# xiexh20/CHORE

Hardware: AMD Instinct MI355X
Metric: query-points/sec (HGFilters encode + 20k-pt MLP field query per 512x512 image) (higher is better)
Workload: dtype fp16x3; 1 GPU; BASELINE configs[1]: encode 4x(5,512,512) + query 4x20000 points per GPU per step; images_per_gpu=4, points_per_image=20000, batches_in_flight=2

## Files before the change

### chore_amd/csrc/query_fwd.hip

```cpp
#include "heads_x3.h"
#include <cstdlib>

template <int PTS>
struct QueryFwdSmemT {
    float X[PTS * XS];
    PtTableT<PTS> tab;
};
using QueryFwdSmem = QueryFwdSmemT<QT_PTS>;

template <typename T, int NCB, bool TRAIN = false, bool X3 = false>
__global__ __launch_bounds__(256, 1) void query_fwd_f32_kernel(QueryArgs a) {
    static_assert(!TRAIN || NCB == 2, "the training staging is written for 64-point tiles");
    constexpr int PTS = 32 * NCB;
    if constexpr (X3) f16_saturate_mode();
    extern __shared__ __attribute__((aligned(16))) char smem_raw[];
    QueryFwdSmemT<PTS>& sm = *reinterpret_cast<QueryFwdSmemT<PTS>*>(smem_raw);
    const int tid = threadIdx.x, lane = tid & 63;
    const int wid = __builtin_amdgcn_readfirstlane(tid >> 6);
    int b, tile_;
    query_block(b, tile_);
    const int n0 = tile_ * PTS;
    const Cam cam{a.fx, a.fy, a.cx, a.cy, a.half_crop, a.crop};

    if (tid < PTS) {
        fill_pt_table(sm.tab, tid, a.points, a.crop_center, b, n0 + tid, a.N, cam, a.FH, a.FW, a.TH,
                      a.TW, nullptr);
        if (a.in_img && n0 + tid < a.N) a.in_img[(size_t)b * a.N + n0 + tid] = (uint8_t)sm.tab.in_img[tid];
    }
    __syncthreads();
    const T* feat_b = (const T*)a.feat + (size_t)b * a.FH * a.FW * FEAT_C;
    const T* tmpx_b = (const T*)a.tmpx + (size_t)b * a.TH * a.TW * TMPX_C;
    gather_tile<T, PTS>(sm.X, sm.tab, feat_b, tmpx_b, wid, lane);
    __syncthreads();

    const float* arena = (const float*)a.arena;
    const int head = wid;
    if constexpr (!TRAIN) {
        if (a.out[head] == nullptr) return;
    }
    f32x16 h1[4][NCB], h2[4][NCB];
    const size_t row0 = (size_t)b * a.N + n0, plane = (size_t)a.B * a.N * HEAD_HID, mplane = (size_t)a.B * a.N * 2;
    if constexpr (TRAIN) {
        for (int i = tid; i < PTS * (QF_KPAD / 4); i += 256) {
            const int pt = i / (QF_KPAD / 4), q = i % (QF_KPAD / 4);
            if (n0 + pt < a.N) *(f32x4*)(a.tX + (row0 + pt) * QF_KPAD + 4 * q) = *(const f32x4*)(sm.X + pt * XS + 4 * q);
        }
    }
    f32x16 o[NCB];
    if constexpr (X3) {
        float inv[NCB];
#pragma unroll
        for (int cb = 0; cb < NCB; ++cb) inv[cb] = QX_INV;
        heads_layer1_x3<NCB>(h1, sm.X, arena, head, lane);
        if constexpr (TRAIN) store_tile<NCB>(a.tH + (0 * HEAD_NUM + head) * plane, h1, true, row0, n0, a.N, lane, 0, inv);
        if constexpr (TRAIN) store_masks<NCB>(a.tM + (0 * HEAD_NUM + head) * mplane, h1, row0, n0, a.N, lane, 0);
        heads_layer_hid_x3<NCB>(h2, h1, arena, head, 1, lane);
        if constexpr (TRAIN) store_tile<NCB>(a.tH + (1 * HEAD_NUM + head) * plane, h2, true, row0, n0, a.N, lane, 0, inv);
        if constexpr (TRAIN) store_masks<NCB>(a.tM + (1 * HEAD_NUM + head) * mplane, h2, row0, n0, a.N, lane, 0);
        heads_layer_hid_x3<NCB>(h1, h2, arena, head, 2, lane);
        if constexpr (TRAIN) store_tile<NCB>(a.tH + (2 * HEAD_NUM + head) * plane, h1, true, row0, n0, a.N, lane, 0, inv);
        if constexpr (TRAIN) store_masks<NCB>(a.tM + (2 * HEAD_NUM + head) * mplane, h1, row0, n0, a.N, lane, 0);
        heads_layer_out_x3<NCB>(o, h1, arena, head, lane);
    } else {
        heads_layer1<NCB>(h1, sm.X, arena, head, lane);
        if constexpr (TRAIN) store_tile<NCB>(a.tH + (0 * HEAD_NUM + head) * plane, h1, true, row0, n0, a.N, lane);
        if constexpr (TRAIN) store_masks<NCB>(a.tM + (0 * HEAD_NUM + head) * mplane, h1, row0, n0, a.N, lane);
        heads_layer_hid<NCB>(h2, h1, arena, head, 1, lane);
        if constexpr (TRAIN) store_tile<NCB>(a.tH + (1 * HEAD_NUM + head) * plane, h2, true, row0, n0, a.N, lane);
        if constexpr (TRAIN) store_masks<NCB>(a.tM + (1 * HEAD_NUM + head) * mplane, h2, row0, n0, a.N, lane);
        heads_layer_hid<NCB>(h1, h2, arena, head, 2, lane);
        if constexpr (TRAIN) store_tile<NCB>(a.tH + (2 * HEAD_NUM + head) * plane, h1, true, row0, n0, a.N, lane);
        if constexpr (TRAIN) store_masks<NCB>(a.tM + (2 * HEAD_NUM + head) * mplane, h1, row0, n0, a.N, lane);
        heads_layer_out<NCB>(o, h1, arena, head, lane);
    }

    const int odim = head_out_dim(head);
    float* outp = a.out[head] + (size_t)b * odim * a.N;
    const int half = lane >> 5, col = lane & 31;
#pragma unroll
    for (int cb = 0; cb < NCB; ++cb) {
        const int pt = cb * 32 + col;
        const int n = n0 + pt;
        const bool inside = sm.tab.in_img[pt] != 0;
#pragma unroll
        for (int r = 0; r < 16; ++r) {
            const int ch = mfma32_row(r, half);
            if (ch < odim && n < a.N) {
                float v = o[cb][r];
                if (head == 0 && !inside) v = 5.0f;
                outp[(size_t)ch * a.N + n] = v;
            }
        }
    }
}

template <typename T, bool TRAIN = false, bool X3 = false>
__global__ __launch_bounds__(512, 1) void query_fwd_f32_w8_kernel(QueryArgs a) {
    constexpr int PTS = 64;
    if constexpr (X3) f16_saturate_mode();
    extern __shared__ __attribute__((aligned(16))) char smem_raw[];
    QueryFwdSmemT<PTS>& sm = *reinterpret_cast<QueryFwdSmemT<PTS>*>(smem_raw);
    const int tid = threadIdx.x, lane = tid & 63;
    const int wid = __builtin_amdgcn_readfirstlane(tid >> 6);
    float* scr = reinterpret_cast<float*>(smem_raw + sizeof(QueryFwdSmemT<PTS>)) + wid * (32 * ST_LD);
    int b, tile_;
    query_block(b, tile_);
    const int n0 = tile_ * PTS;
    const Cam cam{a.fx, a.fy, a.cx, a.cy, a.half_crop, a.crop};
    if (tid < PTS) {
        fill_pt_table(sm.tab, tid, a.points, a.crop_center, b, n0 + tid, a.N, cam, a.FH, a.FW, a.TH,
                      a.TW, nullptr);
        if (a.in_img && n0 + tid < a.N) a.in_img[(size_t)b * a.N + n0 + tid] = (uint8_t)sm.tab.in_img[tid];
    }
    __syncthreads();
    const T* feat_b = (const T*)a.feat + (size_t)b * a.FH * a.FW * FEAT_C;
    const T* tmpx_b = (const T*)a.tmpx + (size_t)b * a.TH * a.TW * TMPX_C;
    gather_tile<T, PTS, 8>(sm.X, sm.tab, feat_b, tmpx_b, wid, lane);
    __syncthreads();

    const float* arena = (const float*)a.arena;
    const int head = wid & 3, cb0 = wid >> 2;
    if constexpr (!TRAIN) {
        if (a.out[head] == nullptr) return;
    }
    f32x16 h1[4][1], h2[4][1];
    const size_t row0 = (size_t)b * a.N + n0, plane = (size_t)a.B * a.N * HEAD_HID, mplane = (size_t)a.B * a.N * 2;
    if constexpr (TRAIN) {
        for (int i = tid; i < PTS * (QF_KPAD / 4); i += 512) {
            const int pt = i / (QF_KPAD / 4), q = i % (QF_KPAD / 4);
            if (n0 + pt < a.N) *(f32x4*)(a.tX + (row0 + pt) * QF_KPAD + 4 * q) = *(const f32x4*)(sm.X + pt * XS + 4 * q);
        }
    }
    f32x16 o[1];
    if constexpr (X3) {
        const float inv[1] = {QX_INV};
        heads_layer1_x3<1>(h1, sm.X + cb0 * 32 * XS, arena, head, lane);
        if constexpr (TRAIN) store_tile_lds<1>(a.tH + (0 * HEAD_NUM + head) * plane, h1, true, row0, n0, a.N, lane, cb0 * 32, inv, scr);
        if constexpr (TRAIN) store_masks<1>(a.tM + (0 * HEAD_NUM + head) * mplane, h1, row0, n0, a.N, lane, cb0 * 32);
        heads_layer_hid_x3<1>(h2, h1, arena, head, 1, lane);
        if constexpr (TRAIN) store_tile_lds<1>(a.tH + (1 * HEAD_NUM + head) * plane, h2, true, row0, n0, a.N, lane, cb0 * 32, inv, scr);
        if constexpr (TRAIN) store_masks<1>(a.tM + (1 * HEAD_NUM + head) * mplane, h2, row0, n0, a.N, lane, cb0 * 32);
        heads_layer_hid_x3<1>(h1, h2, arena, head, 2, lane);
        if constexpr (TRAIN) store_tile_lds<1>(a.tH + (2 * HEAD_NUM + head) * plane, h1, true, row0, n0, a.N, lane, cb0 * 32, inv, scr);
        if constexpr (TRAIN) store_masks<1>(a.tM + (2 * HEAD_NUM + head) * mplane, h1, row0, n0, a.N, lane, cb0 * 32);
        heads_layer_out_x3<1>(o, h1, arena, head, lane);
    } else {
        heads_layer1<1>(h1, sm.X + cb0 * 32 * XS, arena, head, lane);
        if constexpr (TRAIN) store_tile_lds<1>(a.tH + (0 * HEAD_NUM + head) * plane, h1, true, row0, n0, a.N, lane, cb0 * 32, nullptr, scr);
        if constexpr (TRAIN) store_masks<1>(a.tM + (0 * HEAD_NUM + head) * mplane, h1, row0, n0, a.N, lane, cb0 * 32);
        heads_layer_hid<1>(h2, h1, arena, head, 1, lane);
        if constexpr (TRAIN) store_tile_lds<1>(a.tH + (1 * HEAD_NUM + head) * plane, h2, true, row0, n0, a.N, lane, cb0 * 32, nullptr, scr);
        if constexpr (TRAIN) store_masks<1>(a.tM + (1 * HEAD_NUM + head) * mplane, h2, row0, n0, a.N, lane, cb0 * 32);
        heads_layer_hid<1>(h1, h2, arena, head, 2, lane);
        if constexpr (TRAIN) store_tile_lds<1>(a.tH + (2 * HEAD_NUM + head) * plane, h1, true, row0, n0, a.N, lane, cb0 * 32, nullptr, scr);
        if constexpr (TRAIN) store_masks<1>(a.tM + (2 * HEAD_NUM + head) * mplane, h1, row0, n0, a.N, lane, cb0 * 32);
        heads_layer_out<1>(o, h1, arena, head, lane);
    }

    const int odim = head_out_dim(head);
    float* outp = a.out[head] + (size_t)b * odim * a.N;
    const int half = lane >> 5, col = lane & 31;
    const int pt = cb0 * 32 + col, n = n0 + pt;
    const bool inside = sm.tab.in_img[pt] != 0;
#pragma unroll
    for (int r = 0; r < 16; ++r) {
        const int ch = mfma32_row(r, half);
        if (ch < odim && n < a.N) {
            float v = o[0][r];
            if (head == 0 && !inside) v = 5.0f;
            outp[(size_t)ch * a.N + n] = v;
        }
    }
}

constexpr int XSH = 344;
template <int PTS>
struct QuerySplitSmemT {
    static constexpr size_t XB = (size_t)2 * PTS * XSH * 2;
    static constexpr size_t EB = (size_t)HEAD_NUM * 4 * 2 * (PTS / 32) * 2 * 1024;
    __attribute__((aligned(16))) char buf[XB > EB ? XB : EB];
    PtTableT<PTS> tab;
};

template <typename T, int PTS>
__device__ __forceinline__ void gather_tile_split(char* XH, char* XL, const PtTableT<PTS>& tab, const T* feat_b, const T* tmpx_b,
                                                  int wid, int lane) {
    using L = MapLoad<T>;
    constexpr int NW = 8, U = PTS / NW;
    auto put = [&](char* row_h, char* row_l, int k, float v) {
        asm volatile("" : "+v"(v));
        const _Float16 h = (_Float16)v, l = (_Float16)(v - (float)h);
        *(_Float16*)(row_h + 2 * k) = h;
        *(_Float16*)(row_l + 2 * k) = l;
    };
    typename L::Raw4 fv[U][4];
    typename L::Raw1 tv[U][4];
#pragma unroll
    for (int u = 0; u < U; ++u) {
        const int pt = wid * U + u;
#pragma unroll
        for (int k = 0; k < 4; ++k) {
            const int fo = tab.foff[k][pt];
            const int to = tab.toff[k][pt];
            fv[u][k] = (fo >= 0) ? L::raw4(feat_b + fo + lane * 4) : L::zero4();
            tv[u][k] = (to >= 0) ? L::raw1(tmpx_b + to + lane) : L::zero1();
        }
    }
#pragma unroll
    for (int u = 0; u < U; ++u) {
        const int pt = wid * U + u;
        float fw[4], tw[4];
#pragma unroll
        for (int k = 0; k < 4; ++k) { fw[k] = tab.fw[k][pt]; tw[k] = tab.tw[k][pt]; }
        const f32x4 c0 = L::cvt4(fv[u][0]), c1 = L::cvt4(fv[u][1]), c2 = L::cvt4(fv[u][2]), c3 = L::cvt4(fv[u][3]);
        typedef _Float16 h4 __attribute__((ext_vector_type(4)));
        h4 hh, ll;
#pragma unroll
        for (int c = 0; c < 4; ++c) {
            float r = interp4(c0[c], c1[c], c2[c], c3[c], fw);
            asm volatile("" : "+v"(r));
            hh[c] = (_Float16)r;
            ll[c] = (_Float16)(r - (float)hh[c]);
        }
        char* rh = XH + (size_t)pt * XSH * 2;
        char* rl = XL + (size_t)pt * XSH * 2;
        *(h4*)(rh + lane * 8) = hh;
        *(h4*)(rl + lane * 8) = ll;
        put(rh, rl, FEAT_C + 3 + lane, interp4(L::cvt1(tv[u][0], lane & 1), L::cvt1(tv[u][1], lane & 1), L::cvt1(tv[u][2], lane & 1),
                                               L::cvt1(tv[u][3], lane & 1), tw));
        if (lane < 3) put(rh, rl, FEAT_C + lane, tab.xyz[lane][pt]);
        if (lane >= 3 && lane < 3 + (QX_KS1 * 16 - HEAD_IN)) put(rh, rl, HEAD_IN + lane - 3, 0.f);
    }
}

#ifdef CHORE_QUERY_STAMPS
__device__ unsigned long long g_qstamps[4096 * 8];
#define QSTAMP(i) do { if (tid == 0) { const int L_ = blockIdx.x + blockIdx.y * gridDim.x; if (L_ < 4096) g_qstamps[L_ * 8 + (i)] = wall_clock64(); } } while (0)
__device__ unsigned short g_qx[2 * 64 * XSH];
__device__ int g_qx_tile = -1;
extern "C" int chore_debug_query_xdump(unsigned short* out, int tile) {
    if (tile >= 0) return (int)hipMemcpyToSymbol(HIP_SYMBOL(g_qx_tile), &tile, sizeof(int));
    return (int)hipMemcpyFromSymbol(out, HIP_SYMBOL(g_qx), sizeof(unsigned short) * 2 * 64 * XSH);
}
extern "C" int chore_debug_query_stamps(unsigned long long* out, int n) {
    return (int)hipMemcpyFromSymbol(out, HIP_SYMBOL(g_qstamps), sizeof(unsigned long long) * (n < 4096 * 8 ? n : 4096 * 8));
}
#else
#define QSTAMP(i) do { } while (0)
#endif
struct AFrag2 { u32x4 h[2], l[2]; };
__device__ __forceinline__ void load_afrag2(AFrag2& f, const u32x4* A , int rb0) {
#pragma unroll
    for (int i = 0; i < 2; ++i) { f.h[i] = A[((rb0 + i) * 2) * 64]; f.l[i] = A[((rb0 + i) * 2 + 1) * 64]; }
}

template <typename T, int NCB>
__global__ __launch_bounds__(512, 1) void query_fwd_x3_split_kernel(QueryArgs a) {
    constexpr int PTS = 32 * NCB, PF = 7, NSTEP = QX_KS1 + 16;
    static_assert(QX_KS1 % PF == 0, "the k loop of layer 1 is unrolled by the ring depth");
    f16_saturate_mode();
    extern __shared__ __attribute__((aligned(16))) char smem_raw[];
    QuerySplitSmemT<PTS>& sm = *reinterpret_cast<QuerySplitSmemT<PTS>*>(smem_raw);
    char* XH = sm.buf;
    char* XL = sm.buf + (size_t)PTS * XSH * 2;
    u32x4* E = (u32x4*)sm.buf;
    const int tid = threadIdx.x, lane = tid & 63;
    const int wid = __builtin_amdgcn_readfirstlane(tid >> 6);
    const int half = lane >> 5, col = lane & 31;
    int b, tile_;
    query_block(b, tile_);
    const int n0 = tile_ * PTS;
    const Cam cam{a.fx, a.fy, a.cx, a.cy, a.half_crop, a.crop};
    QSTAMP(0);
    if (tid < PTS) {
        fill_pt_table(sm.tab, tid, a.points, a.crop_center, b, n0 + tid, a.N, cam, a.FH, a.FW, a.TH, a.TW, nullptr, a.perm);
        if (a.in_img && n0 + tid < a.N) a.in_img[(size_t)b * a.N + sm.tab.pidx[tid]] = (uint8_t)sm.tab.in_img[tid];
    }
    __syncthreads();
    QSTAMP(1);
    const float* arena = (const float*)a.arena;
    const int head = wid & 3, ch = wid >> 2, rb0 = 2 * ch;
    const bool active = a.out[head] != nullptr;
    const u32x4* xbase = (const u32x4*)((const char*)arena + QX_OFF_BYTES);
    const u32x4* A1 = xbase + (size_t)head * QX_KS1 * 4 * 2 * 64 + lane;
    const u32x4* A23 = xbase + QX_L1_VEC + (size_t)head * 2 * 4 * 2 * 4 * 2 * 64 + lane;
    auto step_ptr = [&](int st) -> const u32x4* {
        return st < QX_KS1 ? A1 + (size_t)st * 4 * 2 * 64 : A23 + (size_t)(st - QX_KS1) * 4 * 2 * 64;
    };
    AFrag2 ring[PF];
    constexpr bool RING_EARLY = sizeof(T) == 2 || NCB == 1;
    if (RING_EARLY && active) {
#pragma unroll
        for (int p = 0; p < PF; ++p) load_afrag2(ring[p], step_ptr(p), rb0);
    }
    const T* feat_b = (const T*)a.feat + (size_t)b * a.FH * a.FW * FEAT_C;
    const T* tmpx_b = (const T*)a.tmpx + (size_t)b * a.TH * a.TW * TMPX_C;
    gather_tile_split<T, PTS>(XH, XL, sm.tab, feat_b, tmpx_b, wid, lane);
    if (!RING_EARLY && active) {
#pragma unroll
        for (int p = 0; p < PF; ++p) load_afrag2(ring[p], step_ptr(p), rb0);
    }
    __syncthreads();
    QSTAMP(2);
#ifdef CHORE_QUERY_STAMPS
    if (b == 0 && tile_ == g_qx_tile)
        for (int i = tid; i < 2 * PTS * XSH; i += 512) g_qx[i] = ((const unsigned short*)sm.buf)[i];
#endif

    f32x16 acc[2][NCB], nb[2];
    auto mm = [&](const AFrag2& f, const u32x4 (&bh)[NCB], const u32x4 (&bl)[NCB]) {
#pragma unroll
        for (int i = 0; i < 2; ++i)
#pragma unroll
            for (int cb = 0; cb < NCB; ++cb) acc[i][cb] = mfma3(f.h[i], f.l[i], bh[cb], bl[cb], acc[i][cb]);
    };
    auto fetch_bias = [&](int layer) {
#pragma unroll
        for (int i = 0; i < 2; ++i) nb[i] = scaled_bias(arena, head, layer, rb0 + i, half);
    };
    auto init_acc = [&]() {
#pragma unroll
        for (int i = 0; i < 2; ++i)
#pragma unroll
            for (int cb = 0; cb < NCB; ++cb) acc[i][cb] = nb[i];
    };
    auto publish = [&]() {
#pragma unroll
        for (int i = 0; i < 2; ++i)
#pragma unroll
            for (int s = 0; s < 2; ++s)
#pragma unroll
                for (int cb = 0; cb < NCB; ++cb) {
                    float v[8];
#pragma unroll
                    for (int j = 0; j < 8; ++j) v[j] = relu(acc[i][cb][8 * s + j] * QX_INV);
                    u32x4 hi, lo;
                    split8(v, hi, lo);
                    u32x4* dst = E + ((((size_t)(head * 4 + rb0 + i) * 2 + s) * NCB + cb) * 2) * 64 + lane;
                    dst[0] = hi;
                    dst[64] = lo;
                }
    };

    if (active) {
        fetch_bias(0);
        init_acc();
        fetch_bias(1);
        const char* xh0 = XH + (size_t)col * XSH * 2 + 16 * half;
        const char* xl0 = XL + (size_t)col * XSH * 2 + 16 * half;
#pragma unroll 1
        for (int k0 = 0; k0 < QX_KS1; k0 += PF) {
#pragma unroll
            for (int p = 0; p < PF; ++p) {
                const int ks = k0 + p;
                u32x4 bh[NCB], bl[NCB];
#pragma unroll
                for (int cb = 0; cb < NCB; ++cb) {
                    bh[cb] = *(const u32x4*)(xh0 + (size_t)cb * 32 * XSH * 2 + ks * 32);
                    bl[cb] = *(const u32x4*)(xl0 + (size_t)cb * 32 * XSH * 2 + ks * 32);
                }
                mm(ring[p], bh, bl);
                load_afrag2(ring[p], step_ptr(ks + PF), rb0);
                __builtin_amdgcn_sched_barrier(0);
            }
        }
    }
    __syncthreads();
    QSTAMP(3);
    if (active) publish();
    __syncthreads();

    u32x4 ah[8], al[8];
#pragma unroll
    for (int layer = 1; layer <= 2; ++layer) {
        if (active) {
            init_acc();
            fetch_bias(layer + 1);
            const u32x4* Eh = E + (size_t)head * 4 * 2 * NCB * 2 * 64 + lane;
#pragma unroll
            for (int t = 0; t < 8; ++t) {
                const int st = QX_KS1 + 8 * (layer - 1) + t;
                u32x4 bh[NCB], bl[NCB];
#pragma unroll
                for (int cb = 0; cb < NCB; ++cb) {
                    bh[cb] = Eh[((size_t)(t * NCB + cb) * 2) * 64];
                    bl[cb] = Eh[((size_t)(t * NCB + cb) * 2 + 1) * 64];
                }
                mm(ring[st % PF], bh, bl);
                if (st + PF < NSTEP) load_afrag2(ring[st % PF], step_ptr(st + PF), rb0);
                __builtin_amdgcn_sched_barrier(0);
            }
            if (layer == 2) {
                const u32x4* A = xbase + QX_L1_VEC + QX_L23_VEC + (size_t)head * 4 * 2 * 2 * 64 + lane;
#pragma unroll
                for (int t = 0; t < 8; ++t) { ah[t] = A[(t * 2) * 64]; al[t] = A[(t * 2 + 1) * 64]; }
            }
        }
        __syncthreads();
        if (active) publish();
        __syncthreads();
    }

    QSTAMP(4);
    const int cb_o = NCB == 2 ? ch : 0;
    if (!active || (NCB == 1 && ch != 0)) return;
    f32x16 o = nb[0];
    if (rb0 != 0) o = scaled_bias(arena, head, 3, 0, half);
    {
        const u32x4* Eh = E + (size_t)head * 4 * 2 * NCB * 2 * 64 + lane;
#pragma unroll
        for (int t = 0; t < 8; ++t) {
            const u32x4 bh = Eh[((size_t)(t * NCB + cb_o) * 2) * 64], bl = Eh[((size_t)(t * NCB + cb_o) * 2 + 1) * 64];
            o = mfma3(ah[t], al[t], bh, bl, o);
        }
    }
    const int odim = head_out_dim(head);
    float* outp = a.out[head] + (size_t)b * odim * a.N;
    const int pt = cb_o * 32 + col, n = sm.tab.pidx[pt];
    const bool inside = sm.tab.in_img[pt] != 0;
#pragma unroll
    for (int r = 0; r < 16; ++r) {
        const int chn = mfma32_row(r, half);
        if (chn < odim && n0 + pt < a.N) {
            float v = o[r] * QX_INV;
            if (head == 0 && !inside) v = 5.0f;
            outp[(size_t)chn * a.N + n] = v;
        }
    }
    QSTAMP(5);
}

template <typename T, int NCB>
static int launch_query_fwd_split(chore_handle* h, const QueryArgs& a, hipStream_t s) {
    constexpr int PTS = 32 * NCB;
    const size_t smem = sizeof(QuerySplitSmemT<PTS>);
    dim3 grid((a.N + PTS - 1) / PTS, a.B);
    return CHORE_LAUNCH(h, s, (query_fwd_x3_split_kernel<T, NCB>), grid, dim3(512), smem, a);
}

template <typename T>
__global__ __launch_bounds__(256) void sample_features_kernel(QueryArgs a, float* features, float* nxy) {
    extern __shared__ __attribute__((aligned(16))) char smem_raw[];
    QueryFwdSmem& sm = *reinterpret_cast<QueryFwdSmem*>(smem_raw);
    const int tid = threadIdx.x, lane = tid & 63;
    const int wid = __builtin_amdgcn_readfirstlane(tid >> 6);
    int b, tile_;
    query_block(b, tile_);
    const int n0 = tile_ * QT_PTS;
    const Cam cam{a.fx, a.fy, a.cx, a.cy, a.half_crop, a.crop};
    if (tid < QT_PTS) {
        float nn[2];
        fill_pt_table(sm.tab, tid, a.points, a.crop_center, b, n0 + tid, a.N, cam, a.FH, a.FW, a.TH, a.TW, nn);
        if (nxy && n0 + tid < a.N) {
            nxy[((size_t)b * a.N + n0 + tid) * 2 + 0] = nn[0];
            nxy[((size_t)b * a.N + n0 + tid) * 2 + 1] = nn[1];
        }
        if (a.in_img && n0 + tid < a.N) a.in_img[(size_t)b * a.N + n0 + tid] = (uint8_t)sm.tab.in_img[tid];
    }
    __syncthreads();
    const T* feat_b = (const T*)a.feat + (size_t)b * a.FH * a.FW * FEAT_C;
    const T* tmpx_b = (const T*)a.tmpx + (size_t)b * a.TH * a.TW * TMPX_C;
    gather_tile<T>(sm.X, sm.tab, feat_b, tmpx_b, wid, lane);
    __syncthreads();
    for (int i = tid; i < QT_PTS * HEAD_IN; i += 256) {
        const int pt = i / HEAD_IN, k = i % HEAD_IN;
        if (n0 + pt < a.N) features[((size_t)b * a.N + n0 + pt) * HEAD_IN + k] = sm.X[pt * XS + k];
    }
}

template <typename T>
static int launch_sample_features_t(chore_handle* h, const QueryArgs& a, float* features, float* nxy, hipStream_t s) {
    const size_t smem = sizeof(QueryFwdSmem);
    dim3 grid((a.N + QT_PTS - 1) / QT_PTS, a.B);
    return CHORE_LAUNCH(h, s, sample_features_kernel<T>, grid, dim3(256), smem, a, features, nxy);
}
int launch_sample_features(chore_handle* h, int dtype, const QueryArgs& a, float* features, float* nxy, hipStream_t s) {
    return dtype == CHORE_F32 ? launch_sample_features_t<float>(h, a, features, nxy, s)
                              : launch_sample_features_t<unsigned short>(h, a, features, nxy, s);
}

__global__ void heads_pack_f32_kernel(HeadsRaw raw, float* arena) {
    const size_t idx = (size_t)blockIdx.x * blockDim.x + threadIdx.x;
    if (idx >= QF_TOTAL_FLOATS) return;
    float v = 0.f;
    if (idx < QF_OFF_L23) {
        size_t t = idx - QF_OFF_L1;
        const int i = t & 3; t >>= 2;
        const int lane = t & 63; t >>= 6;
        const int rb = t & 3; t >>= 2;
        const int q = (int)(t % QF_KG);
        const int h = (int)(t / QF_KG);
        const int row = rb * 32 + (lane & 31);
        const int k = q * 8 + 4 * (lane >> 5) + i;
        if (k < HEAD_IN) v = raw.w[h][0][(size_t)row * HEAD_IN + k];
    } else if (idx < QF_OFF_L4) {
        size_t t = idx - QF_OFF_L23;
        const int i = t & 3; t >>= 2;
        const int lane = t & 63; t >>= 6;
        const int rb = t & 3; t >>= 2;
        const int rg = t & 3; t >>= 2;
        const int kb = t & 3; t >>= 2;
        const int l = t & 1; t >>= 1;
        const int h = (int)t;
        const int row = rb * 32 + (lane & 31);
        const int k = kb * 32 + mfma32_row(rg * 4 + i, lane >> 5);
        v = raw.w[h][1 + l][(size_t)row * HEAD_HID + k];
    } else if (idx < QF_OFF_BIAS) {
        size_t t = idx - QF_OFF_L4;
        const int i = t & 3; t >>= 2;
        const int lane = t & 63; t >>= 6;
        const int rg = t & 3; t >>= 2;
        const int kb = t & 3; t >>= 2;
        const int h = (int)t;
        const int row = lane & 31;
        const int k = kb * 32 + mfma32_row(rg * 4 + i, lane >> 5);
        if (row < head_out_dim(h)) v = raw.w[h][3][(size_t)row * HEAD_HID + k];
    } else if (idx < QB_OFF_L4T) {
        size_t t = idx - QF_OFF_BIAS;
        const int r = t & 15; t >>= 4;
        const int half = t & 1; t >>= 1;
        const int rb = t & 3; t >>= 2;
        const int layer = t & 3; t >>= 2;
        const int h = (int)t;
        const int ch = rb * 32 + mfma32_row(r, half);
        const int dim = (layer == 3) ? head_out_dim(h) : HEAD_HID;
        if (ch < dim) v = raw.b[h][layer][ch];
    } else if (idx < QB_OFF_L32T) {
        size_t t = idx - QB_OFF_L4T;
        const int i = t & 3; t >>= 2;
        const int lane = t & 63; t >>= 6;
        const int rb = t & 3; t >>= 2;
        const int sg = t & 3; t >>= 2;
        const int h = (int)t;
        const int k = 2 * (sg * 4 + i) + (lane >> 5);
        const int in = rb * 32 + (lane & 31);
        if (k < head_out_dim(h)) v = raw.w[h][3][(size_t)k * HEAD_HID + in];
    } else if (idx < QB_OFF_L1T) {
        size_t t = idx - QB_OFF_L32T;
        const int i = t & 3; t >>= 2;
        const int lane = t & 63; t >>= 6;
        const int rb = t & 3; t >>= 2;
        const int rg = t & 3; t >>= 2;
        const int kb = t & 3; t >>= 2;
        const int j = t & 1; t >>= 1;
        const int h = (int)t;
        const int k = kb * 32 + mfma32_row(rg * 4 + i, lane >> 5);
        const int in = rb * 32 + (lane & 31);
        v = raw.w[h][2 - j][(size_t)k * HEAD_HID + in];
    } else {
        size_t t = idx - QB_OFF_L1T;
        const int i = t & 3; t >>= 2;
        const int lane = t & 63; t >>= 6;
        const int rb = (int)(t % QB_RB1); t /= QB_RB1;
        const int rg = t & 3; t >>= 2;
        const int kb = t & 3; t >>= 2;
        const int h = (int)t;
        const int k = kb * 32 + mfma32_row(rg * 4 + i, lane >> 5);
        const int in = rb * 32 + (lane & 31);
        if (in < HEAD_IN) v = raw.w[h][0][(size_t)k * HEAD_IN + in];
    }
    arena[idx] = v;
}

__global__ void heads_pack_x3_kernel(HeadsRaw raw, u32x4* dst) {
    const size_t idx = (size_t)blockIdx.x * blockDim.x + threadIdx.x;
    const size_t n1 = QX_L1_VEC / 2, n23 = QX_L23_VEC / 2, n4 = QX_L4_VEC / 2;
    const size_t n4t = QX_L4T_VEC / 2, n32t = QX_L32T_VEC / 2, n1t = QX_L1T_VEC / 2;
    if (idx >= n1 + n23 + n4 + n4t + n32t + n1t) return;
    float v[8];
    size_t out;
    size_t t = idx;
    const int lane = t & 63, half = lane >> 5;
    if (idx < n1) {
        t >>= 6;
        const int rb = t & 3; t >>= 2;
        const int ks = (int)(t % QX_KS1);
        const int hd = (int)(t / QX_KS1);
        const int row = rb * 32 + (lane & 31);
#pragma unroll
        for (int j = 0; j < 8; ++j) {
            const int k = ks * 16 + 8 * half + j;
            v[j] = k < HEAD_IN ? raw.w[hd][0][(size_t)row * HEAD_IN + k] : 0.f;
        }
        out = (((size_t)hd * QX_KS1 + ks) * 4 + rb) * 2 * 64 + lane;
    } else if (idx < n1 + n23) {
        t = (idx - n1) >> 6;
        const int rb = t & 3; t >>= 2;
        const int s = t & 1; t >>= 1;
        const int kb = t & 3; t >>= 2;
        const int l = t & 1; t >>= 1;
        const int hd = (int)t;
        const int row = rb * 32 + (lane & 31);
#pragma unroll
        for (int j = 0; j < 8; ++j) v[j] = raw.w[hd][1 + l][(size_t)row * HEAD_HID + kb * 32 + mfma32_row(8 * s + j, half)];
        out = QX_L1_VEC + ((((((size_t)hd * 2 + l) * 4 + kb) * 2 + s) * 4 + rb) * 2) * 64 + lane;
    } else if (idx < n1 + n23 + n4) {
        t = (idx - n1 - n23) >> 6;
        const int s = t & 1; t >>= 1;
        const int kb = t & 3; t >>= 2;
        const int hd = (int)t;
        const int row = lane & 31;
#pragma unroll
        for (int j = 0; j < 8; ++j)
            v[j] = row < head_out_dim(hd) ? raw.w[hd][3][(size_t)row * HEAD_HID + kb * 32 + mfma32_row(8 * s + j, half)] : 0.f;
        out = QX_L1_VEC + QX_L23_VEC + ((((size_t)hd * 4 + kb) * 2 + s) * 2) * 64 + lane;
    } else if (idx < n1 + n23 + n4 + n4t) {
        t = (idx - n1 - n23 - n4) >> 6;
        const int rb = t & 3; t >>= 2;
        const int hd = (int)t;
        const int in = rb * 32 + (lane & 31);
#pragma unroll
        for (int j = 0; j < 8; ++j) {
            const int k = 8 * half + j;
            v[j] = k < head_out_dim(hd) ? raw.w[hd][3][(size_t)k * HEAD_HID + in] : 0.f;
        }
        out = QX_OFF_L4T + (((size_t)hd * 4 + rb) * 2) * 64 + lane;
    } else if (idx < n1 + n23 + n4 + n4t + n32t) {
        t = (idx - n1 - n23 - n4 - n4t) >> 6;
        const int rb = t & 3; t >>= 2;
        const int s = t & 1; t >>= 1;
        const int kb = t & 3; t >>= 2;
        const int jl = t & 1; t >>= 1;
        const int hd = (int)t;
        const int in = rb * 32 + (lane & 31);
#pragma unroll
        for (int j = 0; j < 8; ++j) v[j] = raw.w[hd][2 - jl][(size_t)(kb * 32 + mfma32_row(8 * s + j, half)) * HEAD_HID + in];
        out = QX_OFF_L32T + ((((((size_t)hd * 2 + jl) * 4 + kb) * 2 + s) * 4 + rb) * 2) * 64 + lane;
    } else {
        t = (idx - n1 - n23 - n4 - n4t - n32t) >> 6;
        const int rb = (int)(t % QB_RB1); t /= QB_RB1;
        const int s = t & 1; t >>= 1;
        const int kb = t & 3; t >>= 2;
        const int hd = (int)t;
        const int in = rb * 32 + (lane & 31);
#pragma unroll
        for (int j = 0; j < 8; ++j)
            v[j] = in < HEAD_IN ? raw.w[hd][0][(size_t)(kb * 32 + mfma32_row(8 * s + j, half)) * HEAD_IN + in] : 0.f;
        out = QX_OFF_L1T + (((((size_t)hd * 4 + kb) * 2 + s) * QB_RB1 + rb) * 2) * 64 + lane;
    }
#pragma unroll
    for (int j = 0; j < 8; ++j) v[j] *= QX_SCALE;
    u32x4 hi, lo;
    split8(v, hi, lo);
    dst[out] = hi;
    dst[out + 64] = lo;
}

int launch_heads_pack_f32(chore_handle* h, const HeadsRaw& raw, float* arena, hipStream_t s) {
    const int threads = 256;
    const int blocks = (int)((QF_TOTAL_FLOATS + threads - 1) / threads);
    hipLaunchKernelGGL(heads_pack_f32_kernel, dim3(blocks), dim3(threads), 0, s, raw, arena);
    CHORE_LAUNCH_CHECK(h, s);
    const size_t nx = QX_TOTAL_VEC / 2;
    hipLaunchKernelGGL(heads_pack_x3_kernel, dim3((unsigned)((nx + threads - 1) / threads)), dim3(threads), 0, s, raw,
                       (u32x4*)((char*)arena + QX_OFF_BYTES));
    CHORE_LAUNCH_CHECK(h, s);
    return CHORE_OK;
}

size_t heads_arena_bytes() { return QX_ARENA_BYTES; }

template <typename T, int NCB, bool X3 = false>
static int launch_query_fwd_n(chore_handle* h, const QueryArgs& a, hipStream_t s) {
    constexpr int PTS = 32 * NCB;
    const size_t smem = sizeof(QueryFwdSmemT<PTS>);
    dim3 grid((a.N + PTS - 1) / PTS, a.B);
    return CHORE_LAUNCH(h, s, (query_fwd_f32_kernel<T, NCB, false, X3>), grid, dim3(256), smem, a);
}

bool query_small_tiles(int B, int N) { return (size_t)B * ((N + QT_PTS - 1) / QT_PTS) <= 256; }

template <typename T>
static int launch_query_fwd_w8(chore_handle* h, const QueryArgs& a, hipStream_t s) {
    const size_t smem = sizeof(QueryFwdSmemT<64>);
    dim3 grid((a.N + 63) / 64, a.B);
    return CHORE_LAUNCH(h, s, (query_fwd_f32_w8_kernel<T, false, false>), grid, dim3(512), smem, a);
}

static bool query_w4() { static const bool v = getenv("CHORE_QUERY_W4") != nullptr; return v; }

template <typename T, bool X3 = false>
static int launch_query_fwd_t(chore_handle* h, const QueryArgs& a, hipStream_t s) {
    if constexpr (X3) {
        static const bool nosplit = getenv("CHORE_QUERY_X3_NOSPLIT") != nullptr;
        if (!nosplit) return query_small_tiles(a.B, a.N) ? launch_query_fwd_split<T, 1>(h, a, s) : launch_query_fwd_split<T, 2>(h, a, s);
    }
    if (query_small_tiles(a.B, a.N)) return launch_query_fwd_n<T, 1, X3>(h, a, s);
    if constexpr (X3) return launch_query_fwd_n<T, 2, true>(h, a, s);
    else return query_w4() ? launch_query_fwd_n<T, 2>(h, a, s) : launch_query_fwd_w8<T>(h, a, s);
}

template <typename T, bool X3 = false>
static int launch_query_fwd_train_w8(chore_handle* h, const QueryArgs& a, hipStream_t s) {
    const size_t smem = sizeof(QueryFwdSmemT<64>) + 8 * 32 * ST_LD * sizeof(float);
    dim3 grid((a.N + 63) / 64, a.B);
    return CHORE_LAUNCH(h, s, (query_fwd_f32_w8_kernel<T, true, X3>), grid, dim3(512), smem, a);
}

template <typename T, bool X3 = false>
static int launch_query_fwd_train_t(chore_handle* h, const QueryArgs& a, hipStream_t s) {
    if (!query_w4()) return launch_query_fwd_train_w8<T, X3>(h, a, s);
    const size_t smem = sizeof(QueryFwdSmemT<64>);
    dim3 grid((a.N + 63) / 64, a.B);
    return CHORE_LAUNCH(h, s, (query_fwd_f32_kernel<T, 2, true, X3>), grid, dim3(256), smem, a);
}
int launch_query_fwd_train(chore_handle* h, int dtype, const QueryArgs& a, hipStream_t s, int x3) {
    if (x3) return dtype == CHORE_F32 ? launch_query_fwd_train_t<float, true>(h, a, s) : launch_query_fwd_train_t<unsigned short, true>(h, a, s);
    return dtype == CHORE_F32 ? launch_query_fwd_train_t<float>(h, a, s) : launch_query_fwd_train_t<unsigned short>(h, a, s);
}

int launch_query_fwd_f32(chore_handle* h, const QueryArgs& a, hipStream_t s) {
    return launch_query_fwd_t<float>(h, a, s);
}
int launch_query_fwd_f32_bf16maps(chore_handle* h, const QueryArgs& a, hipStream_t s) {
    return launch_query_fwd_t<unsigned short>(h, a, s);
}
int launch_query_fwd_x3(chore_handle* h, int dtype, const QueryArgs& a, hipStream_t s) {
    if (dtype == CHORE_F16) return launch_query_fwd_t<qh16_t, true>(h, a, s);
    return dtype == CHORE_F32 ? launch_query_fwd_t<float, true>(h, a, s) : launch_query_fwd_t<unsigned short, true>(h, a, s);
}
```

Measured before the change: 21.12 million points/s.

## Stream feature gather in chunks through an LDS ring overlapped with layer-1 MFMA

Replaces the up-front gather of the whole tile's sampled features into LDS with a chunked pipeline. Each 32-channel chunk is loaded with buffer loads (out-of-range taps return zero through the buffer resource), interpolated, split into hi/lo fp16 and written into a 4-slot ring, while layer-1 MFMA steps consume earlier chunks. Scheduling barriers interleave the MFMA, LDS and VMEM work. The goal is to hide gather latency behind compute and to shrink the LDS staging footprint. The cost is a much more complex schedule, extra syncthreads per chunk, a smaller weight prefetch ring (3 instead of 7) for NCB=2, and a new 2 GB per-image limit on feature maps.

```diff
diff --git a/chore_amd/csrc/query_fwd.hip b/chore_amd/csrc/query_fwd.hip
--- a/chore_amd/csrc/query_fwd.hip
+++ b/chore_amd/csrc/query_fwd.hip
@@ -173,75 +173,44 @@
     }
 }
 
-constexpr int XSH = 344;
+constexpr int QC_K = 32;
+constexpr int QC_N = (QX_KS1 + 1) / 2;
+constexpr int QC_ROW = 2 * QC_K + 16;
+constexpr int QC_SLOTS = 4;
+constexpr unsigned QC_OOB = 0x80000000u;
 template <int PTS>
 struct QuerySplitSmemT {
-    static constexpr size_t XB = (size_t)2 * PTS * XSH * 2;
+    static constexpr size_t SLOT = (size_t)2 * PTS * QC_ROW;
+    static constexpr size_t XB = QC_SLOTS * SLOT;
     static constexpr size_t EB = (size_t)HEAD_NUM * 4 * 2 * (PTS / 32) * 2 * 1024;
-    __attribute__((aligned(16))) char buf[XB > EB ? XB : EB];
+    static_assert(XB <= EB, "the chunk ring lives inside the exchange area");
+    __attribute__((aligned(16))) char buf[EB];
     PtTableT<PTS> tab;
 };
 
-template <typename T, int PTS>
-__device__ __forceinline__ void gather_tile_split(char* XH, char* XL, const PtTableT<PTS>& tab, const T* feat_b, const T* tmpx_b,
-                                                  int wid, int lane) {
-    using L = MapLoad<T>;
-    constexpr int NW = 8, U = PTS / NW;
-    auto put = [&](char* row_h, char* row_l, int k, float v) {
-        asm volatile("" : "+v"(v));
-        const _Float16 h = (_Float16)v, l = (_Float16)(v - (float)h);
-        *(_Float16*)(row_h + 2 * k) = h;
-        *(_Float16*)(row_l + 2 * k) = l;
-    };
-    typename L::Raw4 fv[U][4];
-    typename L::Raw1 tv[U][4];
-#pragma unroll
-    for (int u = 0; u < U; ++u) {
-        const int pt = wid * U + u;
-#pragma unroll
-        for (int k = 0; k < 4; ++k) {
-            const int fo = tab.foff[k][pt];
-            const int to = tab.toff[k][pt];
-            fv[u][k] = (fo >= 0) ? L::raw4(feat_b + fo + lane * 4) : L::zero4();
-            tv[u][k] = (to >= 0) ? L::raw1(tmpx_b + to + lane) : L::zero1();
-        }
-    }
-#pragma unroll
-    for (int u = 0; u < U; ++u) {
-        const int pt = wid * U + u;
-        float fw[4], tw[4];
-#pragma unroll
-        for (int k = 0; k < 4; ++k) { fw[k] = tab.fw[k][pt]; tw[k] = tab.tw[k][pt]; }
-        const f32x4 c0 = L::cvt4(fv[u][0]), c1 = L::cvt4(fv[u][1]), c2 = L::cvt4(fv[u][2]), c3 = L::cvt4(fv[u][3]);
-        typedef _Float16 h4 __attribute__((ext_vector_type(4)));
-        h4 hh, ll;
-#pragma unroll
-        for (int c = 0; c < 4; ++c) {
-            float r = interp4(c0[c], c1[c], c2[c], c3[c], fw);
-            asm volatile("" : "+v"(r));
-            hh[c] = (_Float16)r;
-            ll[c] = (_Float16)(r - (float)hh[c]);
-        }
-        char* rh = XH + (size_t)pt * XSH * 2;
-        char* rl = XL + (size_t)pt * XSH * 2;
-        *(h4*)(rh + lane * 8) = hh;
-        *(h4*)(rl + lane * 8) = ll;
-        put(rh, rl, FEAT_C + 3 + lane, interp4(L::cvt1(tv[u][0], lane & 1), L::cvt1(tv[u][1], lane & 1), L::cvt1(tv[u][2], lane & 1),
-                                               L::cvt1(tv[u][3], lane & 1), tw));
-        if (lane < 3) put(rh, rl, FEAT_C + lane, tab.xyz[lane][pt]);
-        if (lane >= 3 && lane < 3 + (QX_KS1 * 16 - HEAD_IN)) put(rh, rl, HEAD_IN + lane - 3, 0.f);
-    }
+template <int BYTES>
+__device__ __forceinline__ void qc_load(unsigned* dst, __amdgpu_buffer_rsrc_t rs, unsigned off) {
+    if constexpr (BYTES == 16) {
+        const u32x4 v = __builtin_bit_cast(u32x4, __builtin_amdgcn_raw_buffer_load_b128(rs, (int)off, 0, 0));
+        dst[0] = v[0]; dst[1] = v[1]; dst[2] = v[2]; dst[3] = v[3];
+    } else if constexpr (BYTES == 8) {
+        typedef unsigned u32x2_ __attribute__((ext_vector_type(2)));
+        const u32x2_ v = __builtin_bit_cast(u32x2_, __builtin_amdgcn_raw_buffer_load_b64(rs, (int)off, 0, 0));
+        dst[0] = v[0]; dst[1] = v[1];
+    } else {
+        static_assert(BYTES == 4, "a tap load is 4, 8 or 16 bytes");
+        dst[0] = __builtin_amdgcn_raw_buffer_load_b32(rs, (int)off, 0, 0);
+    }
+}
+template <typename T>
+__device__ __forceinline__ float qc_val(unsigned w, int odd) {
+    if constexpr (sizeof(T) == 4) return __uint_as_float(w);
+    else return MapLoad<T>::cvt1(w, odd);
 }
 
 #ifdef CHORE_QUERY_STAMPS
 __device__ unsigned long long g_qstamps[4096 * 8];
 #define QSTAMP(i) do { if (tid == 0) { const int L_ = blockIdx.x + blockIdx.y * gridDim.x; if (L_ < 4096) g_qstamps[L_ * 8 + (i)] = wall_clock64(); } } while (0)
-__device__ unsigned short g_qx[2 * 64 * XSH];
-__device__ int g_qx_tile = -1;
-extern "C" int chore_debug_query_xdump(unsigned short* out, int tile) {
-    if (tile >= 0) return (int)hipMemcpyToSymbol(HIP_SYMBOL(g_qx_tile), &tile, sizeof(int));
-    return (int)hipMemcpyFromSymbol(out, HIP_SYMBOL(g_qx), sizeof(unsigned short) * 2 * 64 * XSH);
-}
 extern "C" int chore_debug_query_stamps(unsigned long long* out, int n) {
     return (int)hipMemcpyFromSymbol(out, HIP_SYMBOL(g_qstamps), sizeof(unsigned long long) * (n < 4096 * 8 ? n : 4096 * 8));
 }
@@ -256,13 +225,15 @@
 
 template <typename T, int NCB>
 __global__ __launch_bounds__(512, 1) void query_fwd_x3_split_kernel(QueryArgs a) {
-    constexpr int PTS = 32 * NCB, PF = 7, NSTEP = QX_KS1 + 16;
-    static_assert(QX_KS1 % PF == 0, "the k loop of layer 1 is unrolled by the ring depth");
+    constexpr int PTS = 32 * NCB, PF = NCB == 2 ? 3 : 7, NSTEP = QX_KS1 + 16;
+    constexpr int V = 2 * NCB;
+    constexpr int LPP = QC_K / V;
+    constexpr int NMF = 6 * NCB;
+    constexpr size_t SLOT = QuerySplitSmemT<PTS>::SLOT;
+    using L = MapLoad<T>;
     f16_saturate_mode();
     extern __shared__ __attribute__((aligned(16))) char smem_raw[];
     QuerySplitSmemT<PTS>& sm = *reinterpret_cast<QuerySplitSmemT<PTS>*>(smem_raw);
-    char* XH = sm.buf;
-    char* XL = sm.buf + (size_t)PTS * XSH * 2;
     u32x4* E = (u32x4*)sm.buf;
     const int tid = threadIdx.x, lane = tid & 63;
     const int wid = __builtin_amdgcn_readfirstlane(tid >> 6);
@@ -288,24 +259,87 @@
         return st < QX_KS1 ? A1 + (size_t)st * 4 * 2 * 64 : A23 + (size_t)(st - QX_KS1) * 4 * 2 * 64;
     };
     AFrag2 ring[PF];
-    constexpr bool RING_EARLY = sizeof(T) == 2 || NCB == 1;
-    if (RING_EARLY && active) {
-#pragma unroll
-        for (int p = 0; p < PF; ++p) load_afrag2(ring[p], step_ptr(p), rb0);
-    }
-    const T* feat_b = (const T*)a.feat + (size_t)b * a.FH * a.FW * FEAT_C;
-    const T* tmpx_b = (const T*)a.tmpx + (size_t)b * a.TH * a.TW * TMPX_C;
-    gather_tile_split<T, PTS>(XH, XL, sm.tab, feat_b, tmpx_b, wid, lane);
-    if (!RING_EARLY && active) {
-#pragma unroll
-        for (int p = 0; p < PF; ++p) load_afrag2(ring[p], step_ptr(p), rb0);
-    }
-    __syncthreads();
-    QSTAMP(2);
-#ifdef CHORE_QUERY_STAMPS
-    if (b == 0 && tile_ == g_qx_tile)
-        for (int i = tid; i < 2 * PTS * XSH; i += 512) g_qx[i] = ((const unsigned short*)sm.buf)[i];
-#endif
+
+    const int sp = tid / LPP, lq = tid % LPP;
+    const size_t fbytes = (size_t)a.FH * a.FW * FEAT_C * sizeof(T), tbytes = (size_t)a.TH * a.TW * TMPX_C * sizeof(T);
+    auto map_rsrc = [](const void* base, size_t bytes) {
+        const uintptr_t p = (uintptr_t)base;
+        const uintptr_t pu = (uintptr_t)(unsigned)__builtin_amdgcn_readfirstlane((int)(unsigned)p) |
+                             (uintptr_t)(unsigned)__builtin_amdgcn_readfirstlane((int)(unsigned)(p >> 32)) << 32;
+        return __builtin_amdgcn_make_buffer_rsrc((void*)pu, 0, __builtin_amdgcn_readfirstlane((int)bytes), 0x00020000);
+    };
+    const __amdgpu_buffer_rsrc_t frs = map_rsrc((const char*)a.feat + (size_t)b * fbytes, fbytes);
+    const __amdgpu_buffer_rsrc_t trs = map_rsrc((const char*)a.tmpx + (size_t)b * tbytes, tbytes);
+    unsigned fbo[4];
+    float fw[4];
+#pragma unroll
+    for (int k = 0; k < 4; ++k) {
+        const int fo = sm.tab.foff[k][sp];
+        fbo[k] = fo >= 0 ? (unsigned)(fo + V * lq) * (unsigned)sizeof(T) : QC_OOB;
+        fw[k] = sm.tab.fw[k][sp];
+    }
+    auto load_chunk = [&](int c, unsigned (&raw)[4][V]) {
+        if (c < FEAT_C / QC_K) {
+#pragma unroll
+            for (int k = 0; k < 4; ++k) qc_load<V * (int)sizeof(T)>(raw[k], frs, fbo[k] + (unsigned)(c * QC_K * (int)sizeof(T)));
+        } else {
+            unsigned tbo[4];
+#pragma unroll
+            for (int k = 0; k < 4; ++k) {
+                const int to = sm.tab.toff[k][sp];
+                tbo[k] = to >= 0 ? (unsigned)to * (unsigned)sizeof(T) : QC_OOB;
+            }
+#pragma unroll
+            for (int j = 0; j < V; ++j) {
+                int tc = c * QC_K + V * lq + j - (FEAT_C + 3);
+                tc = tc < 0 ? 0 : (tc > TMPX_C - 1 ? TMPX_C - 1 : tc);
+                const unsigned o = ((unsigned)tc * (unsigned)sizeof(T)) & ~3u;
+#pragma unroll
+                for (int k = 0; k < 4; ++k) qc_load<4>(&raw[k][j], trs, tbo[k] + o);
+            }
+        }
+    };
+    auto stage_values = [&](int c, const unsigned (&raw)[4][V], float (&r)[V]) {
+        if (c < FEAT_C / QC_K) {
+#pragma unroll
+            for (int j = 0; j < V; ++j) {
+                const int w = sizeof(T) == 4 ? j : j >> 1;
+                r[j] = interp4(qc_val<T>(raw[0][w], j & 1), qc_val<T>(raw[1][w], j & 1), qc_val<T>(raw[2][w], j & 1),
+                               qc_val<T>(raw[3][w], j & 1), fw);
+            }
+        } else {
+            float tw[4];
+#pragma unroll
+            for (int k = 0; k < 4; ++k) tw[k] = sm.tab.tw[k][sp];
+#pragma unroll
+            for (int j = 0; j < V; ++j) {
+                const int odd = (j + 1) & 1;
+                r[j] = interp4(qc_val<T>(raw[0][j], odd), qc_val<T>(raw[1][j], odd), qc_val<T>(raw[2][j], odd), qc_val<T>(raw[3][j], odd), tw);
+                const int kk = c * QC_K + V * lq + j;
+                if (c == FEAT_C / QC_K) {
+                    const float xv = sm.tab.xyz[kk - FEAT_C < 2 ? kk - FEAT_C : 2][sp];
+                    r[j] = kk < FEAT_C + 3 ? xv : r[j];
+                }
+                if (c == QC_N - 1) r[j] = kk < HEAD_IN ? r[j] : 0.f;
+            }
+        }
+    };
+    auto pin_values = [&](float (&r)[V]) {
+#pragma unroll
+        for (int j = 0; j < V; ++j) asm volatile("" : "+v"(r[j]));
+    };
+    auto split_write = [&](int c, const float (&r)[V]) {
+        typedef _Float16 hv __attribute__((ext_vector_type(V)));
+        hv hh, ll;
+#pragma unroll
+        for (int j = 0; j < V; ++j) {
+            hh[j] = (_Float16)r[j];
+            ll[j] = (_Float16)(r[j] - (float)hh[j]);
+        }
+        char* row = sm.buf + (size_t)(c % QC_SLOTS) * SLOT + (size_t)sp * QC_ROW + lq * V * 2;
+        *(hv*)row = hh;
+        *(hv*)(row + (size_t)PTS * QC_ROW) = ll;
+    };
 
     f32x16 acc[2][NCB], nb[2];
     auto mm = [&](const AFrag2& f, const u32x4 (&bh)[NCB], const u32x4 (&bl)[NCB]) {
@@ -341,39 +375,95 @@
                     dst[64] = lo;
                 }
     };
-
-    if (active) {
-        fetch_bias(0);
-        init_acc();
-        fetch_bias(1);
-        const char* xh0 = XH + (size_t)col * XSH * 2 + 16 * half;
-        const char* xl0 = XL + (size_t)col * XSH * 2 + 16 * half;
+    const char* xrow = sm.buf + (size_t)col * QC_ROW + 16 * half;
+    u32x4 xbh[2][NCB], xbl[2][NCB];
+    auto read_b = [&](int ks) {
+        const char* x = xrow + (size_t)((ks >> 1) % QC_SLOTS) * SLOT + (ks & 1) * 32;
+#pragma unroll
+        for (int cb = 0; cb < NCB; ++cb) {
+            xbh[ks & 1][cb] = *(const u32x4*)(x + (size_t)cb * 32 * QC_ROW);
+            xbl[ks & 1][cb] = *(const u32x4*)(x + (size_t)(PTS + cb * 32) * QC_ROW);
+        }
+    };
+    auto kstep1 = [&](int ks) {
+        mm(ring[ks % PF], xbh[ks & 1], xbl[ks & 1]);
+        load_afrag2(ring[ks % PF], step_ptr(ks + PF), rb0);
+    };
+
+    unsigned raw[2][4][V];
+    float r[V];
+    auto first_chunks = [&](auto act_) {
+        if constexpr (decltype(act_)::value) {
+#pragma unroll
+            for (int p = 0; p < PF; ++p) load_afrag2(ring[p], step_ptr(p), rb0);
+        }
+        load_chunk(0, raw[0]);
+        load_chunk(1, raw[1]);
+        if constexpr (decltype(act_)::value) {
+            fetch_bias(0);
+            init_acc();
+        }
+        stage_values(0, raw[0], r);
+        load_chunk(2, raw[0]);
+        pin_values(r);
+        split_write(0, r);
+        stage_values(1, raw[1], r);
+        load_chunk(3, raw[1]);
+        __syncthreads();
+        if constexpr (decltype(act_)::value) read_b(0);
+    };
+
+    auto layer1 = [&](auto act_) {
+        constexpr bool ACT = decltype(act_)::value;
+#pragma unroll
+        for (int c = 0; c < QC_N; ++c) {
+            if (ACT && 2 * c + 1 < QX_KS1) read_b(2 * c + 1);
+            if (c + 1 < QC_N) pin_values(r);
+            if constexpr (ACT) kstep1(2 * c);
+            if (c + 1 < QC_N) split_write(c + 1, r);
+#pragma unroll
+            for (int i = 0; i < NMF; ++i) {
+                if constexpr (ACT) __builtin_amdgcn_sched_group_barrier(0x008, 1, 0);
+                if (ACT && i < 2 * NCB) __builtin_amdgcn_sched_group_barrier(0x100, 1, 0);
+                __builtin_amdgcn_sched_group_barrier(0x002, 3, 0);
+                if constexpr (ACT) __builtin_amdgcn_sched_group_barrier(0x020, 1, 0);
+            }
+            __builtin_amdgcn_sched_barrier(0);
+            __syncthreads();
+            if (2 * c + 1 >= QX_KS1) break;
+            if (ACT && 2 * c + 2 < QX_KS1) read_b(2 * c + 2);
+            if constexpr (ACT) kstep1(2 * c + 1);
+            if (c + 2 < QC_N) stage_values(c + 2, raw[c & 1], r);
+            if (c + 4 < QC_N) load_chunk(c + 4, raw[c & 1]);
+            if (ACT && c == QC_N - 2) fetch_bias(1);
+#pragma unroll
+            for (int i = 0; i < NMF; ++i) {
+                if constexpr (ACT) __builtin_amdgcn_sched_group_barrier(0x008, 1, 0);
+                if (ACT && i < 2 * NCB) __builtin_amdgcn_sched_group_barrier(0x100, 1, 0);
+                __builtin_amdgcn_sched_group_barrier(0x002, 3, 0);
+                __builtin_amdgcn_sched_group_barrier(0x020, 2, 0);
+            }
+            __builtin_amdgcn_sched_barrier(0);
+        }
+    };
+    if (!active) {
+        first_chunks(std::false_type{});
+        layer1(std::false_type{});
 #pragma unroll 1
-        for (int k0 = 0; k0 < QX_KS1; k0 += PF) {
-#pragma unroll
-            for (int p = 0; p < PF; ++p) {
-                const int ks = k0 + p;
-                u32x4 bh[NCB], bl[NCB];
-#pragma unroll
-                for (int cb = 0; cb < NCB; ++cb) {
-                    bh[cb] = *(const u32x4*)(xh0 + (size_t)cb * 32 * XSH * 2 + ks * 32);
-                    bl[cb] = *(const u32x4*)(xl0 + (size_t)cb * 32 * XSH * 2 + ks * 32);
-                }
-                mm(ring[p], bh, bl);
-                load_afrag2(ring[p], step_ptr(ks + PF), rb0);
-                __builtin_amdgcn_sched_barrier(0);
-            }
-        }
-    }
+        for (int i = 0; i < 5; ++i) __syncthreads();
+        return;
+    }
+    first_chunks(std::true_type{});
+    QSTAMP(2);
+    layer1(std::true_type{});
+    QSTAMP(3);
+    publish();
     __syncthreads();
-    QSTAMP(3);
-    if (active) publish();
-    __syncthreads();
 
     u32x4 ah[8], al[8];
 #pragma unroll
     for (int layer = 1; layer <= 2; ++layer) {
-        if (active) {
+        {
             init_acc();
             fetch_bias(layer + 1);
             const u32x4* Eh = E + (size_t)head * 4 * 2 * NCB * 2 * 64 + lane;
@@ -397,13 +487,13 @@
             }
         }
         __syncthreads();
-        if (active) publish();
+        publish();
         __syncthreads();
     }
 
     QSTAMP(4);
     const int cb_o = NCB == 2 ? ch : 0;
-    if (!active || (NCB == 1 && ch != 0)) return;
+    if (NCB == 1 && ch != 0) return;
     f32x16 o = nb[0];
     if (rb0 != 0) o = scaled_bias(arena, head, 3, 0, half);
     {
@@ -419,10 +509,10 @@
     const int pt = cb_o * 32 + col, n = sm.tab.pidx[pt];
     const bool inside = sm.tab.in_img[pt] != 0;
 #pragma unroll
-    for (int r = 0; r < 16; ++r) {
-        const int chn = mfma32_row(r, half);
+    for (int r_ = 0; r_ < 16; ++r_) {
+        const int chn = mfma32_row(r_, half);
         if (chn < odim && n0 + pt < a.N) {
-            float v = o[r] * QX_INV;
+            float v = o[r_] * QX_INV;
             if (head == 0 && !inside) v = 5.0f;
             outp[(size_t)chn * a.N + n] = v;
         }
@@ -434,6 +524,8 @@
 static int launch_query_fwd_split(chore_handle* h, const QueryArgs& a, hipStream_t s) {
     constexpr int PTS = 32 * NCB;
     const size_t smem = sizeof(QuerySplitSmemT<PTS>);
+    if ((size_t)a.FH * a.FW * FEAT_C * sizeof(T) >= QC_OOB || (size_t)a.TH * a.TW * TMPX_C * sizeof(T) >= QC_OOB)
+        CHORE_FAIL(h, CHORE_EINVAL, "query forward: a feature map of %d x %d / %d x %d texels is beyond 2 GB per image", a.FH, a.FW, a.TH, a.TW);
     dim3 grid((a.N + PTS - 1) / PTS, a.B);
     return CHORE_LAUNCH(h, s, (query_fwd_x3_split_kernel<T, NCB>), grid, dim3(512), smem, a);
 }
```

Measured after the change: 21.12 million points/s (median of 3 runs). Within noise of the previous version (+0.0%).
